# richardbaihe/a3t

Measured on AMD Instinct MI355X. Metric: mel-frames/sec (train), higher is better.
Workload: dtype bf16; 1 GPU; VCTK A3T masked-mel train step: 6+6 Conformer blocks d=384 H=2 ff=1536(k3), B=32/GPU, T_mel=1000, T_phn=120, postnet 5x256x5, fwd+bwd+clip+Adam, dropout 0.2/0.2/0.2 + postnet 0.5 (recipe); global_batch=32, parallelism=dp1, params=100799808

## Files before the change

a3t_amd/_lib.py:

```python
import ctypes
import os
from ctypes import POINTER, c_char_p, c_float, c_int, c_int32, c_int64, c_void_p

import torch

HERE = os.path.dirname(os.path.abspath(__file__))
LIB_PATH = os.environ.get("A3T_LIB_PATH") or os.path.join(HERE, "lib", "liba3t_hip.so")

F32, BF16 = 0, 1
ACT_NONE, ACT_RELU, ACT_TANH, ACT_SWISH = 0, 1, 2, 3
ACC_STORE, ACC_ADD, ACC_ATOMIC, ACC_SOLE = 0, 1, 2, 3


class GemmDesc(ctypes.Structure):
    _fields_ = [
        ("A", c_void_p), ("B", c_void_p), ("C", c_void_p), ("bias", c_void_p), ("R", c_void_p), ("S", c_void_p),
        ("M", c_int32), ("N", c_int32), ("K", c_int32),
        ("a_rs", c_int64), ("a_cs", c_int64),
        ("b_rs", c_int64), ("b_cs", c_int64), ("b_ts", c_int64),
        ("c_rs", c_int64),
        ("batch", c_int32), ("batch_inner", c_int32),
        ("a_bs0", c_int64), ("a_bs1", c_int64), ("b_bs0", c_int64), ("b_bs1", c_int64),
        ("c_bs0", c_int64), ("c_bs1", c_int64),
        ("taps", c_int32), ("pad", c_int32), ("dil", c_int32), ("Tseq", c_int32), ("kshift", c_int32),
# ... 35 lines not shown
    "a3t_attn_scale_rows": [_P, _P, _P, c_int, c_int, c_int, c_int, _P],
    "a3t_attn_bwd_ds": [_P, _P, _P, _P, _P, _P, _P, c_int, c_int, c_int, c_int, c_int64, c_int64, c_int64, c_int64, c_float,
                        c_float, ctypes.c_uint32, c_int, c_int64, _P],
    "a3t_attn_fwd": [_P, _P, _P, _P, _P, _P, _P, _P, c_int, c_int, c_int, c_int, c_int64, c_int64, c_int64, c_int64,
                     c_float, c_float, ctypes.c_uint32, _P, _P, _P],
    "a3t_pwg_block": [_P, _P, _P, _P, _P, _P, _P, _P, c_int, c_int, c_int, _P],
    "a3t_mask_fill": [_P, _P, _P, _P, c_int, c_int, c_int, _P],
    "a3t_embed_finish_fwd": [_P, _P, _P, _P, _P, _P, _P, c_int, c_int, c_int, c_int, c_float, c_float, ctypes.c_uint32,
                             _P, _P],
    "a3t_embed_finish_bwd": [_P, _P, _P, _P, _P, _P, _P, _P, c_int, c_int, c_int, c_int, c_int, c_int, c_float, c_float,
                             ctypes.c_uint32, _P],
    "a3t_scale": [_P, _P, c_int64, c_float, _P],
    "a3t_axpy": [_P, _P, c_int64, c_float, _P],
    "a3t_attn_bias_fold": [_P, c_int32, c_int32, _P, _P, _P, _P],
    "a3t_scale_dev": [_P, _P, c_int64, _P, _P],
    "a3t_slice_rows": [_P, _P, c_int, c_int, c_int, c_int, c_int, c_int, _P],
    "a3t_concat_rows": [_P, _P, _P, c_int, c_int, c_int, c_int, _P],
    "a3t_concat_rows_ragged": [_P, _P, _P, _P, _P, c_int, c_int, c_int, c_int, c_int64, c_int64, _P],
    "a3t_split_rows": [_P, _P, _P, c_int, c_int, c_int, c_int, _P],
    "a3t_cast_bf16": [_P, _P, c_int64, _P],
    "a3t_cast_bf16_conv_t": [_P, _P, _P, _P, c_int, c_int, c_int, c_int, _P],
    "a3t_split_bf16": [_P, _P, _P, c_int64, _P],
    "a3t_reflect_pad": [_P, _P, c_int, c_int, c_int, c_int, _P],
    "a3t_reflect_pad_ragged": [_P, _P, _P, c_int, c_int, c_int, c_int, _P],
    "a3t_stft_amp": [_P, _P, c_int64, c_int, c_int, _P],
    "a3t_logmel_finish": [_P, _P, c_int, c_int, c_int, _P],
    "a3t_mlm_loss": [_P, _P, _P, _P, _P, _P, _P, _P, c_int, c_int, c_int, c_float, _P],
    "a3t_mlm_loss_scratch_floats": [c_int],
    "a3t_sumsq": [_P, c_int64, _P, _P],
    "a3t_clip_adam": [_P, _P, _P, _P, _P, _P, c_int64, c_float, c_float, c_float, c_float, c_int, c_float, c_float,
                      _P],
    "a3t_clip_adam_noam": [_P, _P, _P, _P, _P, _P, c_int64, _P, c_float, c_float, c_float, c_float, c_float, c_float,
                           c_float, c_float, _P],
    "a3t_sgd_step": [_P, _P, c_int64, c_float, c_float, _P],
    "a3t_pwg_gate": [_P, _P, _P, c_int64, c_int, _P],
    "a3t_pwg_res_skip": [_P, _P, _P, c_int64, c_int, c_int, _P],
    "a3t_pwg_upsample": [_P, _P, _P, c_int64, c_int64, c_int, c_int, _P],
    "a3t_replicate_pad": [_P, _P, c_int64, c_int64, c_int, c_int, _P],
    "a3t_bias_act": [_P, _P, c_int64, c_int, c_int, c_float, _P],
    "a3t_replicate_pad_ragged": [_P, _P, _P, c_int64, c_int64, c_int, c_int, _P],
    "a3t_pwg_upsample_ragged": [_P, _P, _P, _P, c_int, c_int64, c_int64, c_int, c_int, _P],
    "a3t_zero_tail": [_P, _P, c_int, c_int64, c_int64, c_int, _P],
    "a3t_layernorm_fwd_ragged": [_P, _P, _P, _P, _P, _P, _P, c_int, c_int, c_int, c_float, _P],
    "a3t_glu_dwconv_fwd_ragged": [_P, _P, _P, _P, _P, _P, c_int, c_int, c_int, c_int, _P],
    "a3t_relpos_softmax_fwd_ragged": [_P, _P, c_int, _P, _P, c_int, c_int, c_int, c_int, c_int64, c_int64, c_int64, c_float,
                                      _P],
    "a3t_splice_spans": [_P, _P, _P, _P, _P, _P, c_int, c_int, c_int, c_int, _P],
    "a3t_pwg_block_ragged": [_P, _P, _P, _P, _P, _P, _P, _P, _P, c_int, c_int, c_int, c_int, _P],
    "a3t_pwg_block_f16": [_P, _P, _P, _P, _P, _P, _P, _P, _P, c_int, c_int, c_int, c_int, _P],
    "a3t_cast_f16_sat": [_P, _P, c_int64, _P],
    "a3t_hfg_conv": [_P, _P, _P, _P, _P, _P, c_float, c_int, c_float, _P, c_int, c_int, c_int, c_int, c_int, c_int, _P],
    "a3t_hfg_conv_f16": [_P, _P, _P, _P, _P, _P, c_float, c_int, c_float, _P, c_int, c_int, c_int, c_int, c_int, c_int, _P],
    "a3t_hfg_out": [_P, _P, _P, _P, c_float, _P, c_int, c_int, c_int, c_int, c_int, _P],
    "a3t_leaky_relu": [_P, _P, c_int64, c_float, _P],
    "a3t_mgan_stack": [_P, _P, _P, _P, c_float, _P, c_int, c_int, c_int, c_int, c_int, c_int, _P],
    "a3t_mgan_out": [_P, _P, _P, _P, c_float, c_int, _P, c_int, c_int, c_int, c_int, c_int, c_int, c_int, _P],
    "a3t_pqmf_synthesis": [_P, _P, _P, _P, c_int, c_int, c_int, c_int, c_int, _P],
    "a3t_reflect_pad_rows": [_P, _P, c_int64, c_int64, c_int, c_int, _P],
    "a3t_reflect_pad_rows_ragged": [_P, _P, _P, c_int, c_int64, c_int64, c_int, c_int, _P],
    "a3t_smg_conv": [_P, _P, _P, _P, _P, _P, _P, c_int, c_int, _P, c_int, c_int, c_int, c_int, c_int, c_int, c_int, c_int, c_int,
                     c_int, _P],
    "a3t_smg_stats": [_P, _P, _P, c_float, _P, c_int, c_int, c_int, c_int, _P],
    "a3t_duration_head": [_P, _P, _P, _P, _P, _P, _P, c_int, c_int, c_float, c_float, _P],
    "a3t_l2_normalize": [_P, _P, c_int, c_int, c_float, _P],
    "a3t_gst_conv_bn_relu": [_P, _P, _P, _P, _P, _P, c_int, c_int, c_int, c_int, c_int, c_int, c_int, _P],
    "a3t_gst_gru_stl": [_P, _P, _P, _P, _P, _P, _P, _P, _P, _P, _P, _P, c_int, c_int, c_int, c_int, c_int, c_int, _P],
# ... 57 lines not shown
```

a3t_amd/conformer.py:

```python
import math
import os
import zlib
from dataclasses import dataclass

import torch

from . import ops
from ._lib import ACC_ADD, ACC_ATOMIC, ACC_STORE, ACT_RELU, ACT_SWISH, BF16, F32
from .config import A3TConfig
from .params import ParamStore
from .schedule import StepSchedule


def legacy_pe_table(c: A3TConfig) -> torch.Tensor:
    d = c.adim
    position = torch.arange(c.max_len - 1, -1, -1.0, dtype=torch.float32).unsqueeze(1)
    div = torch.exp(torch.arange(0, d, 2, dtype=torch.float32) * -(math.log(10000.0) / d))
    pe = torch.zeros(c.max_len, d)
    pe[:, 0::2] = torch.sin(position * div)
    pe[:, 1::2] = torch.cos(position * div)
    return pe


def score_chunks(lengths, heads, max_score_elems):
    order = sorted(range(len(lengths)), key=lambda i: (lengths[i], i))
    out, cur = [], []
    for i in order:
        if cur and (len(cur) + 1) * heads * lengths[i] ** 2 > max_score_elems:
            out.append(cur)
            cur = []
        cur.append(i)
    if cur:
        out.append(cur)
    return out


@dataclass
class EngineOptions:
    side_stream: bool = True
    side2: bool = True
    side_depth: int = 48
    wgrad_group: bool = True
    post_f32_first: bool = True
    attn_bwd_ds: bool = True
    attn_signed: bool = True
    attn_dq_dual: bool = True
    attn_dbd_view: bool = True
    attn_dk_main: bool = True
    fused_attn: str = "auto"
    fused_attn_train: int = 1
    ffn_8p: bool = True
    ffn_keep4: bool = True
    lin_dgrad_t: bool = True
    fuse_ln_dropout: bool = True

    @classmethod
    def from_env(cls, environ=os.environ):
        fa, ft = environ.get("A3T_FUSED_ATTN", "auto"), environ.get("A3T_FUSED_ATTN_TRAIN", "1")
        if fa not in ("auto", "fwd", "0"):
            raise ValueError(f"A3T_FUSED_ATTN={fa!r}: expected auto, fwd or 0 (the flash backward behind '1' left the library in "
                             "round 5, tools/experiments/attn_flash_backward.patch)")
        on = {f: environ.get("A3T_" + f.upper(), "1") != "0" for f in
              ("side_stream", "side2", "wgrad_group", "post_f32_first", "attn_bwd_ds", "attn_signed", "attn_dq_dual",
               "attn_dbd_view", "attn_dk_main", "ffn_8p", "ffn_keep4", "lin_dgrad_t")}
        return cls(side_depth=max(2, int(environ.get("A3T_SIDE_DEPTH", "48"))), fused_attn=fa,
                   fused_attn_train=0 if ft == "0" else 2 if ft == "2" else 1, **on)


class ConformerStack(StepSchedule):
    def __init__(self, cfg: A3TConfig, store: ParamStore, compute: str = "f32", training: bool = True,
                 dropout: bool = False, options: EngineOptions = None):
        self.opt = opt = options if options is not None else EngineOptions.from_env()
        super().__init__(store.device, opt.side_stream, opt.side2, opt.side_depth)
        self.c = cfg
        self.dropping = bool(dropout and training)
        self.step_seed = 0
        self.store = store
        self.bf16 = (compute == "bf16")
        self.adt = torch.bfloat16 if self.bf16 else torch.float32
        self.cmp = BF16 if self.bf16 else F32
        self.training = training
        self.pe = legacy_pe_table(cfg).to(self.dev)
        self.sv = {}
        self.scratch64 = torch.zeros(4 * max(cfg.ff, 3 * cfg.adim, cfg.postnet_chans, 64), dtype=torch.float64,
                                     device=self.dev)
        self.bn_momentum = 0.1
        self._wg_group = 4 if (self.bf16 and self.side is not None and self._depth >= 8 and opt.wgrad_group) else 1
        self._wg_pending, self._wg_slots = [], set()
        self._gm_ready = None
        self.colsum_slots = 16
        self.fused_attn_fwd_only = self.bf16 and opt.fused_attn == "fwd"
        self.fused_attn_auto = self.bf16 and opt.fused_attn == "auto"
        self.fused_attn_train = self.bf16 and opt.fused_attn == "auto" and opt.fused_attn_train != 0
        self.fused_attn_train_min = 1 if opt.fused_attn_train == 2 else 64
        self._fused_now = self._fused_train_now = False
        self.attn_path, self.block_dims = {}, {}
        self._need_grad = training
        self._mode_tag = None
        if self.bf16:
            for n, v in (("adim", cfg.adim), ("ff", cfg.ff), ("idim", cfg.idim), ("odim", cfg.odim),
                         ("dk", cfg.dk), ("postnet_chans", cfg.postnet_chans or 8)):
                if v % 8:
                    raise ValueError(f"compute='bf16' needs {n} % 8 == 0 (16-byte DMA granules), got {v}")
            self.flat16 = torch.zeros(store.total, dtype=torch.bfloat16, device=self.dev)
            self.p16 = {k: self.flat16[o:o + math.prod(s)].view(s) for k, (o, s) in store.offsets.items()}
        self._ffn_plans = {}
        self._lin_plans = {}
        self._wt = {}
        self._P_ahead, self._pos_ev = {}, None
        self._cast_ev = self._wt_ev = None
        dec = [o for k, (o, _) in store.offsets.items() if k.startswith("dec.")]
        self._cast_split = min(dec) if dec else 0

    def _drop(self, p, tag):
        if not self.dropping or p <= 0.0:
            return None
        h = (zlib.crc32(tag.encode()) ^ ((self.step_seed * 0x9E3779B1) & 0xFFFFFFFF)) & 0xFFFFFFFF
        h = ((h ^ (h >> 16)) * 0x85EBCA6B) & 0xFFFFFFFF
        h = ((h ^ (h >> 13)) * 0xC2B2AE35) & 0xFFFFFFFF
        return (float(p), (h ^ (h >> 16)) & 0xFFFFFFFF)

    def _gm(self, g, tag, p, bias_grad, bias_scale):
        dr = self._drop(p, tag)
        if dr is None:
            return (self._g16(g) if self.bf16 else g)
        gm = self.ws.get(self._t("tmp.gm"), tuple(g.shape), self.adt)
        if self._gm_ready == tag:
            self._gm_ready = None
            return gm
        ops.dropout_bwd_cast(g, gm, dr[0], dr[1], colsum=bias_grad, colsum_scale=bias_scale)
        return gm

    def W(self, name):
        return self.p16[name] if self.bf16 else self.store.p[name]

    def refresh_weights(self):
        self._cast_ev = self._wt_ev = None
        if not self.bf16:
            return
        split = self._cast_split if self.side is not None else 0
        flat, flat16 = self.store.flat, self.flat16
        wt = list(self._wt.values()) if self._need_grad else []

        def transposed():
            for src_off, dst_off, _, tflat, shp in wt:
                ops.cast_bf16_conv_t(flat, tflat, src_off, dst_off, *shp)
        if split <= 0:
            ops.cast_bf16(flat, flat16)
            transposed()
            return
        ops.cast_bf16(flat[:split], flat16[:split])
        self._cast_ev = self._side(lambda: ops.cast_bf16(flat[split:], flat16[split:]), want_event="cast")
        if wt:
            self._wt_ev = self._side(transposed, want_event="wt")

    def _wait_cast(self, which):
        ev = getattr(self, which, None)
        if ev is not None:
            ev.wait_on(torch.cuda.current_stream())
            setattr(self, which, None)

    def _setup_wt(self, suf, shape):
        stored = (tuple(shape), (shape[0], shape[2])) if shape[1] == 1 else (tuple(shape),)
        names = [k for k in self.store.offsets if k.endswith("." + suf) and tuple(self.store.offsets[k][1]) in stored]
        if not names:
            return
        n = math.prod(shape)
        flat = torch.zeros(n * len(names), dtype=torch.bfloat16, device=self.dev)
        src = torch.tensor([self.store.offsets[k][0] for k in names], dtype=torch.int64, device=self.dev)
        dst = torch.arange(len(names), dtype=torch.int64, device=self.dev) * n
        views = {k: flat[i * n:(i + 1) * n].view(shape[2], shape[1], shape[0]) for i, k in enumerate(names)}
        self._wt[suf] = (src, dst, views, flat, tuple(shape))
        ops.cast_bf16_conv_t(self.store.flat, flat, src, dst, *shape)

    def _ffn_plan(self, M):
        key = (M, self._need_grad, self._mode_tag, self.opt.ffn_8p, self.opt.ffn_keep4)
        if key not in self._ffn_plans:
            c = self.c
            keep = d1 = d2 = keep4 = False
            if self._need_grad and self.bf16 and self.dev.type == "cuda" and self.opt.ffn_8p:
                k = c.ff_kernel
                drop = ops.G8_DROP if (self.dropping and c.dropout_rate > 0) else 0
                keep = ops.gemm_8p_supported(M, c.ff, k * c.adim, k, ops.G8_BIAS_ACT | drop | ops.G8_KEEP_OUT) and \
                    ops.gemm_8p_supported(M, c.ff, k * c.adim, k, ops.G8_KEEP_IN | ops.G8_COLSUM)
                d1 = ops.gemm_8p_supported(M, c.adim, k * c.ff, k, 0) or ops.gemm_pn_supported(M, c.adim, k * c.ff, k, 0)
                d2 = (not keep) and \
                    ops.gemm_pn_supported(M, c.ff, k * c.adim, k, ops.G8_SMASK | ops.G8_COLSUM)
                keep4 = (not keep) and self.opt.ffn_keep4 and c.ff % 8 == 0 and \
                    ops.gemm_pn_supported(M, c.ff, k * c.adim, k, ops.G8_KEEP_IN | ops.G8_COLSUM)
                d2 = d2 or keep4
                if (keep or d2) and "w2" not in self._wt:
                    self._setup_wt("w2", (c.adim, k, c.ff))
                if d1 and "w1" not in self._wt:
                    self._setup_wt("w1", (c.ff, k, c.adim))
                keep, d1, d2 = keep and "w2" in self._wt, d1 and "w1" in self._wt, d2 and "w2" in self._wt
                keep4 = keep4 and d2
            self._ffn_plans[key] = (keep, d1, d2, keep4)
# ... 472 lines not shown
```

a3t_amd/csrc/misc.hip:

```cpp
#include <hip/hip_runtime.h>
#include <math.h>
#include <stdint.h>
#include "../../include/a3t_hip.h"
#include "dtype_io.h"

static inline int nblocks(int64_t n, int cap = 4096) {
    int64_t b = (n + 255) / 256;
    return (int)(b > cap ? cap : (b < 1 ? 1 : b));
}
#define GRID_STRIDE(i, n) \
    for (int64_t i = (int64_t)blockIdx.x * blockDim.x + threadIdx.x; i < (n); i += (int64_t)gridDim.x * blockDim.x)

__global__ void mask_fill_kernel(const float* __restrict__ x, const uint8_t* __restrict__ m,
                                 const float* __restrict__ mf, void* __restrict__ y, int y_dt, int64_t n, int C) {
    GRID_STRIDE(i, n) {
        int64_t r = i / C;
        int c = (int)(i - r * C);
        stx(y, y_dt, i, m[r] ? mf[c] : x[i]);
    }
}
extern "C" int a3t_mask_fill(const float* speech, const uint8_t* masked, const float* mask_feature, void* out,
                             int out_dtype, int M, int C, void* stream) {
    int64_t n = (int64_t)M * C;
    hipLaunchKernelGGL(mask_fill_kernel, dim3(nblocks(n)), dim3(256), 0, (hipStream_t)stream, speech, masked,
// ... 480 lines not shown
    __shared__ double red[256];
    double s = 0.0;
    for (int i = threadIdx.x; i < SUMSQ_BLOCKS; i += 256) s += partial[i];
    red[threadIdx.x] = s;
    __syncthreads();
    for (int o = 128; o > 0; o >>= 1) {
        if (threadIdx.x < o) red[threadIdx.x] += red[threadIdx.x + o];
        __syncthreads();
    }
    const float norm = (float)sqrt(red[0]) * fabsf(gscale);
    if (blockIdx.x == 0 && threadIdx.x == 0) norm_out[0] = norm;
    if (!isfinite(norm)) return;
    const double t = (double)(state[0] + 1);
    const float lr = (float)((double)base_lr * pow((double)model_size, -0.5) * fmin(pow(t, -0.5), t * pow((double)warmup, -1.5)));
    const float bc1 = (float)(1.0 - pow((double)b1, t));
    const float bc2s = (float)sqrt(1.0 - pow((double)b2, t));
    float coef = clip > 0.f ? clip / (norm + 1e-6f) : 1.f;
    coef = (coef > 1.f ? 1.f : coef) * gscale;
    const float step_size = lr / bc1;
    adam_sweep(p, g, m, v, n, coef, b1, b2, step_size, bc2s, eps);
}
__global__ void adam_state_advance_kernel(const float* norm, int* state) {
    if (isfinite(norm[0])) state[0] += 1; else state[1] += 1;
}
extern "C" int a3t_clip_adam_noam(float* p, const float* g, float* m, float* v, const double* partial, float* norm_out,
                                  int64_t n, int* state, float base_lr, float model_size, float warmup, float beta1,
                                  float beta2, float eps, float clip, float gscale, void* stream) {
    hipLaunchKernelGGL(clip_adam_noam_kernel, dim3(nblocks(n / 4, 2048)), dim3(256), 0, (hipStream_t)stream, p, g, m, v,
                       partial, norm_out, n, state, base_lr, model_size, warmup, beta1, beta2, eps, clip, gscale);
    hipLaunchKernelGGL(adam_state_advance_kernel, dim3(1), dim3(1), 0, (hipStream_t)stream, norm_out, state);
    return (int)hipGetLastError();
}

__global__ __launch_bounds__(256) void sgd_step_kernel(float* __restrict__ p, const float* __restrict__ g, const int64_t n,
                                                       const float step) {
    const int64_t tid = (int64_t)blockIdx.x * blockDim.x + threadIdx.x, nthr = (int64_t)gridDim.x * blockDim.x;
    const bool vec = ((((uintptr_t)p) | ((uintptr_t)g)) & 15) == 0;
    const int64_t n4 = vec ? n / 4 : 0;
    for (int64_t i = tid; i < n4; i += nthr) {
        float4 pi = ((float4*)p)[i];
        const float4 gi = ((const float4*)g)[i];
        pi.x -= step * gi.x, pi.y -= step * gi.y, pi.z -= step * gi.z, pi.w -= step * gi.w;
        ((float4*)p)[i] = pi;
    }
    for (int64_t i = n4 * 4 + tid; i < n; i += nthr) p[i] -= step * g[i];
}
extern "C" int a3t_sgd_step(float* p, const float* g, int64_t n, float lr, float gscale, void* stream) {
    if (n <= 0) return 0;
    hipLaunchKernelGGL(sgd_step_kernel, dim3(nblocks((n + 3) / 4, 2048)), dim3(256), 0, (hipStream_t)stream, p, g, n,
                       lr * gscale);
    return (int)hipGetLastError();
}

__global__ void pwg_gate_kernel(const float* __restrict__ y, const float* __restrict__ c, float* __restrict__ out,
                                int64_t n, int H) {
    GRID_STRIDE(i, n) {
        int64_t t = i / H;
        int h = (int)(i - t * H);
        int64_t j = t * 2 * H + h;
        float a = y[j] + c[j], b = y[j + H] + c[j + H];
        out[i] = tanhf(a) * (1.f / (1.f + __expf(-b)));
    }
}
extern "C" int a3t_pwg_gate(const float* y, const float* c, float* out, int64_t T, int H, void* stream) {
    int64_t n = T * H;
    hipLaunchKernelGGL(pwg_gate_kernel, dim3(nblocks(n)), dim3(256), 0, (hipStream_t)stream, y, c, out, n, H);
// ... 259 lines not shown
```

a3t_amd/ops.py:

```python
import ctypes
import os

import torch

from . import _lib as L
from ._lib import ACC_ADD, ACC_ATOMIC, ACC_SOLE, ACC_STORE, ACT_NONE, ACT_RELU, ACT_SWISH, ACT_TANH, BF16, F32

__all__ = ["gemm", "gemm_plan", "linear_fwd", "linear_bwd_data", "linear_bwd_weight", "conv_fwd", "conv_bwd_data",
           "conv_bwd_weight"]


PROFILE = None


def _stream():
    return ctypes.c_void_p(torch.cuda.current_stream().cuda_stream)


def _ptr(t):
    if t is None:
        return None
    return ctypes.c_void_p(t.data_ptr())


# ... 423 lines not shown
    host_lens = [int(n) for n in host_lens]
    if len(host_lens) != B or lens.numel() != B:
        raise ValueError(f"reflect_pad_ragged: {B} rows, {len(host_lens)} host lengths, {lens.numel()} device lengths")
    for b, n in enumerate(host_lens):
        if n <= pad or n > N:
            raise ValueError(f"reflect_pad_ragged: row {b} has {n} samples; reflection by {pad} needs {pad} < n <= {N}")
    L.check(L.load().a3t_reflect_pad_ragged(_ptr(x), _ptr(out), _ptr(_i32(lens, "lens")), B, N, pad, out.shape[1], _stream()),
            "reflect_pad_ragged")


def stft_amp(S, amp, nbins):
    L.check(L.load().a3t_stft_amp(_ptr(S), _ptr(amp), amp.shape[0], nbins, amp.shape[1], _stream()), "stft_amp")


def logmel_finish(mel, olens, B, F, C):
    L.check(L.load().a3t_logmel_finish(_ptr(mel), _ptr(olens), B, F, C, _stream()), "logmel_finish")


def mlm_loss(before, after, target, masked, loss_out, d_before, d_after, scratch, l2=False, gscale=1.0):
    M, C = before.shape
    L.check(L.load().a3t_mlm_loss(_ptr(before), _ptr(after), _ptr(target), _ptr(masked), _ptr(loss_out),
                                  _ptr(d_before), _ptr(d_after), _ptr(scratch), M, C, int(l2), gscale, _stream()),
            "mlm_loss")


def loss_scratch_floats(M):
    return L.load().a3t_mlm_loss_scratch_floats(M)


def sumsq(g, partial):
    L.check(L.load().a3t_sumsq(_ptr(g), g.numel(), _ptr(partial), _stream()), "sumsq")


def clip_adam(p, g, m, v, partial, norm_out, lr, step, clip=1.0, gscale=1.0, betas=(0.9, 0.999), eps=1e-8):
    L.check(L.load().a3t_clip_adam(_ptr(p), _ptr(g), _ptr(m), _ptr(v), _ptr(partial), _ptr(norm_out), p.numel(), lr,
                                   betas[0], betas[1], eps, step, clip, gscale, _stream()), "clip_adam")


def clip_adam_noam(p, g, m, v, partial, norm_out, state, base_lr, model_size, warmup, clip=1.0, gscale=1.0,
                   betas=(0.9, 0.999), eps=1e-8):
    L.check(L.load().a3t_clip_adam_noam(_ptr(p), _ptr(g), _ptr(m), _ptr(v), _ptr(partial), _ptr(norm_out), p.numel(),
                                        _ptr(state), base_lr, float(model_size), float(warmup), betas[0], betas[1], eps,
                                        clip, gscale, _stream()), "clip_adam_noam")


def sgd_step(p, g, lr, gscale=1.0):
    if p.dtype != torch.float32 or g.dtype != torch.float32 or p.numel() != g.numel() or not (p.is_contiguous() and g.is_contiguous()):
        raise ValueError("sgd_step: p and g must be contiguous fp32 buffers of one size")
    L.check(L.load().a3t_sgd_step(_ptr(p), _ptr(g), p.numel(), float(lr), float(gscale), _stream()), "sgd_step")


def pwg_gate(y, c, out):
    T, H = out.shape
    L.check(L.load().a3t_pwg_gate(_ptr(y), _ptr(c), _ptr(out), T, H, _stream()), "pwg_gate")


def pwg_res_skip(o, x, skips):
    T, R = x.shape
    L.check(L.load().a3t_pwg_res_skip(_ptr(o), _ptr(x), _ptr(skips), T, R, skips.shape[1], _stream()), "pwg_res_skip")


def _i32(t, what):
    if t.dtype != torch.int32 or not t.is_contiguous():
        raise ValueError(f"{what} must be a contiguous int32 tensor")
    return t


def _rows_lens(what, x, lens):
    B = x.shape[0] if x.dim() == 3 else 1
    if lens is not None and _i32(lens, "lens").numel() != B:
        raise ValueError(f"{what}: {lens.numel()} lengths for {B} rows")
    return (B, *x.shape[-2:])


def pwg_upsample(c, w, out, scale_, lens=None, mul=1):
    B, Tin, C = _rows_lens("pwg_upsample", c, lens)
    if lens is None:
        rc = L.load().a3t_pwg_upsample(_ptr(c), _ptr(w), _ptr(out), B, Tin, C, scale_, _stream())
    else:
        rc = L.load().a3t_pwg_upsample_ragged(_ptr(c), _ptr(w), _ptr(out), _ptr(lens), mul, B, Tin, C, scale_, _stream())
    L.check(rc, "pwg_upsample")

# ... 393 lines not shown
```

a3t_amd/trainer.py:

```python
import os
from typing import Dict, List, Sequence

import torch
import torch.distributed as dist

from .config import A3TConfig


def shard_batches(batches: Sequence[Sequence[str]], rank: int, world: int) -> List[List[str]]:
    for b in batches:
        if len(b) < world:
            raise RuntimeError(f"The batch-size must be equal or more than world_size: {len(b)} < {world}")
    return [list(b[rank::world]) for b in batches]


def noam_lr(step: int, base_lr: float, model_size: int, warmup: int) -> float:
    return base_lr * model_size ** -0.5 * min(step ** -0.5, step * warmup ** -1.5)


def iterator_stop(local_done: bool, device="cpu") -> bool:
    if not (dist.is_available() and dist.is_initialized()):
        return local_done
    t = torch.tensor([1 if local_done else 0], dtype=torch.int64, device=device)
    dist.all_reduce(t, op=dist.ReduceOp.SUM)
# ... 64 lines not shown
    def wait(self):
        for w, rng in self.works:
            if rng is None:
                w.wait()
                continue
            if self.cuda:
                with torch.cuda.stream(self.stream):
                    w.wait()
                    self.g[rng[0]:rng[1]].copy_(self.stage[rng[0]:rng[1]])
            else:
                w.wait()
                self.g[rng[0]:rng[1]].copy_(self.stage[rng[0]:rng[1]])
        self.works = []
        if self.cuda:
            torch.cuda.current_stream().wait_stream(self.stream)


class A3TTrainer:

    def __init__(self, cfg: A3TConfig, store, compute="bf16", lr=1.0, warmup_steps=4000, grad_clip=1.0,
                 betas=(0.9, 0.999), eps=1e-8, overlap=True, dropout=True, force_reducer=False,
                 bucket_min_elems=16 * 1024 * 1024, comm_dtype=torch.float32):
        from .engine import MLMEngine
        self.cfg, self.store = cfg, store
        self.engine = MLMEngine(cfg, store, compute=compute, training=True, dropout=dropout)
        dev = store.device
        self.m = torch.zeros_like(store.flat)
        self.v = torch.zeros_like(store.flat)
        self.partial = torch.zeros(1024, dtype=torch.float64, device=dev)
        self.norm = torch.zeros(1, device=dev)
        self.step_no = 0
        self.opt_state = torch.zeros(2, dtype=torch.int32, device=dev)
        self.comm_dtype = comm_dtype
        self.lr, self.warmup, self.clip, self.betas, self.eps = lr, warmup_steps, grad_clip, betas, eps
        self.world = dist.get_world_size() if (dist.is_available() and dist.is_initialized()) else 1
        self._main = None
        if dev.type == "cuda":
            from .schedule import shared_stream
            self._main = shared_stream(dev, "main", high=True)
        self.reducer = None
        if self.world > 1 or (force_reducer and dist.is_available() and dist.is_initialized()):
            dist.broadcast(store.flat, 0)
            for b in store.buf.values():
                dist.broadcast(b, 0)
            bounds = [store.offsets[f"pre.{i}.ffm.ln.g"][0] for i in range(cfg.pre_blocks)]
            bounds += [store.offsets[f"enc.{i}.ffm.ln.g"][0] for i in range(cfg.enc_blocks)]
            bounds += [store.offsets[f"dec.{i}.ffm.ln.g"][0] for i in range(cfg.dec_blocks if cfg.has_decoder else 0)]
            bounds += [store.offsets["sfc.w"][0]]
            self.ranges = bucket_ranges(store.total, bounds, bucket_min_elems)
            if overlap:
                self.reducer = FlatAllReduce(store.grad, self.ranges, comm_dtype)

    def step(self, batch: Dict[str, torch.Tensor], total_weight: float = None, accum_grad: int = 1,
             accum_index: int = 0) -> torch.Tensor:
        if self._main is None:
            return self._step(batch, total_weight, accum_grad, accum_index)
        cur = torch.cuda.current_stream(self.store.device)
        self._main.wait_stream(cur)
        with torch.cuda.stream(self._main):
            loss = self._step(batch, total_weight, accum_grad, accum_index)
        cur.wait_stream(self._main)
        loss.record_stream(cur)
        return loss

    def _step(self, batch: Dict[str, torch.Tensor], total_weight: float = None, accum_grad: int = 1,
              accum_index: int = 0) -> torch.Tensor:
        from . import ops
        st = self.store
        if accum_index == 0:
            st.zero_grad()
        if self.engine.bf16:
            from .espnet_model import ESPnetMLMEncAsDecoderModel
            batch = ESPnetMLMEncAsDecoderModel._pad_to_dma_granule(batch)
        w = 1.0
        if total_weight is not None:
            w = grad_scale(float(batch["speech"].shape[0]), float(total_weight), self.world)
        out = self.engine.forward(batch, gscale=w / accum_grad)
        last = (accum_index == accum_grad - 1)
        if self.reducer is not None and last:
            self._backward_overlapped()
        else:
            self.engine.backward()
            if self.world > 1 and last:
                dist.all_reduce(st.grad)
        if not last:
            return out["loss"]
        self.step_no += 1
        ops.sumsq(st.grad, self.partial)
        ops.clip_adam_noam(st.flat, st.grad, self.m, self.v, self.partial, self.norm, self.opt_state, self.lr,
                           self.cfg.adim, self.warmup, clip=self.clip, gscale=1.0 / self.world, betas=self.betas,
                           eps=self.eps)
        return out["loss"]

    def optimizer_steps(self):
        a, sk = self.opt_state.tolist()
        if sk:
            import logging
            logging.warning(f"{sk} step(s) had a non-finite gradient norm and were skipped (trainer.py:640-645)")
        return a, sk

    def _backward_overlapped(self):
        eng, red = self.engine, self.reducer
        state = {"next": 0}
        lows = [lo for lo, _ in red.ranges]
        offs = self.store.offsets

        def after(name):
            lo = offs[name][0]
            if state["next"] < len(lows) and lows[state["next"]] >= lo and hasattr(eng, "join_side"):
                eng.join_side()
            while state["next"] < len(lows) and lows[state["next"]] >= lo:
                red.reduce_range(state["next"])
                state["next"] += 1

        eng.backward(on_group_done=after)
        while state["next"] < len(lows):
            red.reduce_range(state["next"])
            state["next"] += 1
        red.wait()

    def state(self):
        applied = int(self.opt_state[0])
        return dict(model=self.store.state_dict(), optimizers=[dict(m=self.m.cpu(), v=self.v.cpu(), step=applied)],
                    schedulers=[dict(step=applied, warmup_steps=self.warmup)], reporter=None, scaler=None)
# ... 10 lines not shown
```

include/a3t_hip.h:

```cpp
#ifndef A3T_HIP_H
#define A3T_HIP_H
#include <stdint.h>

#ifdef __cplusplus
extern "C" {
#endif

#define A3T_F32 0
#define A3T_BF16 1

#define A3T_EINVAL (-22)

#define A3T_ACT_NONE 0
#define A3T_ACT_RELU 1
#define A3T_ACT_TANH 2
#define A3T_ACT_SWISH 3

#define A3T_ACC_STORE 0
#define A3T_ACC_ADD 1
#define A3T_ACC_ATOMIC 2
#define A3T_ACC_SOLE 3

typedef struct a3t_gemm_desc {
    const void* A;
// ... 104 lines not shown
int a3t_axpy(const float* x, float* y, int64_t n, float a, void* stream);
int a3t_attn_bias_fold(const float* slots, int S, int d, float* gu, float* gv, float* gbqkv, void* stream);
int a3t_scale_dev(const float* x, float* y, int64_t n, const float* s, void* stream);
int a3t_slice_rows(const float* x, void* y, int y_dtype, int B, int T, int Tm, int D, int reverse_add,
                   void* stream);
int a3t_concat_rows(const float* speech, const float* text, float* xs, int B, int Tm, int Tp, int D, void* stream);
int a3t_split_rows(const float* dxs, float* dspeech, float* dtext, int B, int Tm, int Tp, int D, void* stream);
int a3t_concat_rows_ragged(const float* speech, const float* text, float* xs, const int32_t* slens, const int32_t* tlens, int B,
                           int Tm, int Tp, int D, int64_t speech_bs, int64_t text_bs, void* stream);
int a3t_cast_bf16(const float* x, void* y, int64_t n, void* stream);
int a3t_cast_bf16_conv_t(const float* src, void* dst, const int64_t* src_off, const int64_t* dst_off, int count, int N,
                         int taps, int C, void* stream);
int a3t_split_bf16(const float* x, void* hi, void* lo, int64_t n, void* stream);

int a3t_reflect_pad(const float* x, float* out, int B, int N, int pad, int ld, void* stream);
int a3t_reflect_pad_ragged(const float* x, float* out, const int32_t* lens, int B, int N, int pad, int ld, void* stream);
int a3t_stft_amp(const float* S, float* amp, int64_t rows, int nbins, int ld, void* stream);
int a3t_logmel_finish(float* mel, const int64_t* olens, int B, int F, int C, void* stream);

int a3t_mlm_loss(const float* before, const float* after, const float* target, const uint8_t* masked,
                 float* loss_out, float* d_before, float* d_after, float* scratch, int M, int C, int l2,
                 float gscale, void* stream);
int a3t_mlm_loss_scratch_floats(int M);

int a3t_sumsq(const float* g, int64_t n, double* partial , void* stream);
int a3t_clip_adam(float* p, const float* g, float* m, float* v, const double* partial, float* norm_out,
                  int64_t n, float lr, float beta1, float beta2, float eps, int step, float clip,
                  float gscale, void* stream);

int a3t_clip_adam_noam(float* p, const float* g, float* m, float* v, const double* partial, float* norm_out, int64_t n,
                       int32_t* state, float base_lr, float model_size, float warmup, float beta1, float beta2,
                       float eps, float clip, float gscale, void* stream);

int a3t_sgd_step(float* p, const float* g, int64_t n, float lr, float gscale, void* stream);

int a3t_pwg_gate(const float* y, const float* c, float* out, int64_t T, int H, void* stream);
int a3t_pwg_res_skip(const float* o, float* x, float* skips, int64_t T, int R, int S, void* stream);
int a3t_pwg_upsample(const float* c, const float* w, float* out, int64_t B, int64_t Tin, int C, int scale,
                     void* stream);
int a3t_replicate_pad(const float* x, float* y, int64_t B, int64_t T, int C, int pad, void* stream);
int a3t_bias_act(float* x, const float* bias, int64_t M, int C, int act, float scale, void* stream);
int a3t_replicate_pad_ragged(const float* x, float* y, const int32_t* lens, int64_t B, int64_t T, int C, int pad,
                             void* stream);
int a3t_pwg_upsample_ragged(const float* c, const float* w, float* out, const int32_t* lens, int mul, int64_t B,
                            int64_t Tin, int C, int scale, void* stream);
int a3t_zero_tail(float* x, const int32_t* lens, int mul, int64_t B, int64_t T, int C, void* stream);
int a3t_layernorm_fwd_ragged(const float* x, const float* gamma, const float* beta, float* y, float* mean, float* rstd,
                             const int32_t* lens, int B, int T, int D, float eps, void* stream);
int a3t_glu_dwconv_fwd_ragged(const float* g, const float* wdw, const float* bdw, float* glu, float* z, const int32_t* lens,
                              int B, int Tseq, int C, int K, void* stream);
int a3t_relpos_softmax_fwd_ragged(const void* ac, const void* bd, int scores_dtype, const int32_t* lens, void* probs,
                                  int probs_dtype, int B, int H, int T, int64_t ac_bs, int64_t bd_bs, int64_t p_bs,
                                  float scale, void* stream);
int a3t_splice_spans(const float* after, const float* speech, const uint8_t* speech_mask, const int32_t* spans, float* out,
                     int32_t* lens, int B, int Tin, int Tout, int C, void* stream);

int a3t_duration_head(const float* z, const float* gamma, const float* beta, const float* w, const float* bias,
                      float* logd, int64_t* frames, int M, int C, float eps, float offset, void* stream);
int a3t_l2_normalize(const float* x, float* y, int B, int n, float eps, void* stream);

int a3t_gst_conv_bn_relu(const float* x, const float* w, const float* scale, const float* shift, float* y,
                         const int32_t* lens, int B, int Tin, int Fin, int Cin, int Cout, int k, int s, void* stream);
int a3t_gst_gru_stl(const float* gi, const float* w_hh, const float* b_hh, const int32_t* lens, const float* w_q,
                    const float* b_q, const float* k_tok, const float* v_tok, const float* w_out, const float* b_out,
                    float* ref_embs, float* style, int B, int T, int H, int d, int heads, int tokens, void* stream);
int a3t_gst_add_style(float* hs, const float* style, const int32_t* rows, int B, int T, int d, int S, void* stream);
// ... 71 lines not shown
```

Measured before the change: 780,200 mel-frames/s.

## Fuse bf16 weight shadow and transposed-weight casts into the Adam update kernel

The Adam step now writes the bf16 copy of each parameter and the transposed/tap-reversed bf16 weight shadows straight from registers, using a tile table that maps flat regions to transposed destinations. The next step's separate cast and transpose pass is skipped when a version token shows the fp32 buffer is unchanged since the optimizer wrote it. This removes one full read of the fp32 parameter buffer and extra kernel launches each step. In exchange it adds an LDS-tiled transpose inside the optimizer kernel, host-side table validation, and staleness tracking through tensor version counters.

```diff
diff --git a/a3t_amd/_lib.py b/a3t_amd/_lib.py
--- a/a3t_amd/_lib.py
+++ b/a3t_amd/_lib.py
@@ -91,6 +91,9 @@
                       _P],
     "a3t_clip_adam_noam": [_P, _P, _P, _P, _P, _P, c_int64, _P, c_float, c_float, c_float, c_float, c_float, c_float,
                            c_float, c_float, _P],
+    "a3t_adam_shadow_table": [_P, c_int, c_int64, _P],
+    "a3t_clip_adam_noam_shadow": [_P, _P, _P, _P, _P, _P, c_int64, _P, c_float, c_float, c_float, c_float, c_float, c_float,
+                                  c_float, c_float, _P, _P, _P, c_int, _P],
     "a3t_sgd_step": [_P, _P, c_int64, c_float, c_float, _P],
     "a3t_pwg_gate": [_P, _P, _P, c_int64, c_int, _P],
     "a3t_pwg_res_skip": [_P, _P, _P, c_int64, c_int, c_int, _P],
diff --git a/a3t_amd/conformer.py b/a3t_amd/conformer.py
--- a/a3t_amd/conformer.py
+++ b/a3t_amd/conformer.py
@@ -53,6 +53,7 @@
     ffn_keep4: bool = True
     lin_dgrad_t: bool = True
     fuse_ln_dropout: bool = True
+    adam_shadows = True
 
     @classmethod
     def from_env(cls, environ=os.environ):
@@ -63,8 +64,47 @@
         on = {f: environ.get("A3T_" + f.upper(), "1") != "0" for f in
               ("side_stream", "side2", "wgrad_group", "post_f32_first", "attn_bwd_ds", "attn_signed", "attn_dq_dual",
                "attn_dbd_view", "attn_dk_main", "ffn_8p", "ffn_keep4", "lin_dgrad_t")}
-        return cls(side_depth=max(2, int(environ.get("A3T_SIDE_DEPTH", "48"))), fused_attn=fa,
-                   fused_attn_train=0 if ft == "0" else 2 if ft == "2" else 1, **on)
+        opt = cls(side_depth=max(2, int(environ.get("A3T_SIDE_DEPTH", "48"))), fused_attn=fa,
+                  fused_attn_train=0 if ft == "0" else 2 if ft == "2" else 1, **on)
+        opt.adam_shadows = environ.get("A3T_ADAM_SHADOWS", "1") != "0"
+        return opt
+
+
+def shadow_group_names(offsets, suf, shape):
+    stored = (tuple(shape), (shape[0], shape[2])) if shape[1] == 1 else (tuple(shape),)
+    return [k for k in offsets if k.endswith("." + suf) and tuple(offsets[k][1]) in stored]
+
+
+def shadow_set_id(wt):
+    return tuple((suf, id(g[3])) for suf, g in wt.items())
+
+
+def shadow_regions(offsets, wt):
+    out = []
+    for _, _, views, tflat, (N, taps, C) in wt.values():
+        for i, name in enumerate(views):
+            out.append((offsets[name][0], tflat, i * N * taps * C, N, taps, C))
+    return sorted(out, key=lambda r: r[0])
+
+
+def shadow_remainder(regions, total):
+    out, end = [], 0
+    for src, _, _, N, taps, C in regions:
+        if src > end:
+            out.append((end, src))
+        end = src + N * taps * C
+    if total > end:
+        out.append((end, total))
+    return out
+
+
+class ShadowToken:
+
+    def __init__(self, flat, set_id):
+        self.ptr, self.version, self.set_id = flat.data_ptr(), flat._version, set_id
+
+    def valid(self, flat, set_id):
+        return self.ptr == flat.data_ptr() and self.version == flat._version and self.set_id == set_id
 
 
 class ConformerStack(StepSchedule):
@@ -109,6 +149,7 @@
         self._wt = {}
         self._P_ahead, self._pos_ev = {}, None
         self._cast_ev = self._wt_ev = None
+        self._fresh = None
         dec = [o for k, (o, _) in store.offsets.items() if k.startswith("dec.")]
         self._cast_split = min(dec) if dec else 0
 
@@ -138,6 +179,9 @@
         self._cast_ev = self._wt_ev = None
         if not self.bf16:
             return
+        if self.shadows_fresh():
+            return
+        self._fresh = None
         split = self._cast_split if self.side is not None else 0
         flat, flat16 = self.store.flat, self.flat16
         wt = list(self._wt.values()) if self._need_grad else []
@@ -154,6 +198,13 @@
         if wt:
             self._wt_ev = self._side(transposed, want_event="wt")
 
+    def shadows_written(self):
+        self._fresh = ShadowToken(self.store.flat, shadow_set_id(self._wt))
+
+    def shadows_fresh(self):
+        return bool(self.bf16 and self.opt.adam_shadows and self._fresh is not None and
+                    self._fresh.valid(self.store.flat, shadow_set_id(self._wt)))
+
     def _wait_cast(self, which):
         ev = getattr(self, which, None)
         if ev is not None:
@@ -161,8 +212,7 @@
             setattr(self, which, None)
 
     def _setup_wt(self, suf, shape):
-        stored = (tuple(shape), (shape[0], shape[2])) if shape[1] == 1 else (tuple(shape),)
-        names = [k for k in self.store.offsets if k.endswith("." + suf) and tuple(self.store.offsets[k][1]) in stored]
+        names = shadow_group_names(self.store.offsets, suf, shape)
         if not names:
             return
         n = math.prod(shape)
diff --git a/a3t_amd/csrc/misc.hip b/a3t_amd/csrc/misc.hip
--- a/a3t_amd/csrc/misc.hip
+++ b/a3t_amd/csrc/misc.hip
@@ -536,6 +536,187 @@
     return (int)hipGetLastError();
 }
 
+#define SHT 64
+enum { SH_SRC = 0, SH_DST, SH_DOFF, SH_N, SH_TAPS, SH_C, SH_FLAT0, SH_TILE0 };
+static_assert(A3T_SHADOW_COLS == 8 && A3T_SHADOW_FLAT == 4096, "table row, flat tile = 256 lanes x 4 float4");
+static inline int64_t sh_cdiv(int64_t a, int64_t b) { return (a + b - 1) / b; }
+static bool shadow_row(const int64_t* e, bool closing, int64_t n, int64_t& end, int64_t& tile) {
+    const int64_t src = e[SH_SRC], N = e[SH_N], taps = e[SH_TAPS], C = e[SH_C];
+    if (src < end || src % 4 || src > n) return false;
+    if (e[SH_FLAT0] != end || e[SH_TILE0] != tile) return false;
+    tile += sh_cdiv(src - end, A3T_SHADOW_FLAT);
+    if (closing) return src == n && !N && !taps && !C;
+    if (N <= 0 || taps <= 0 || C <= 0 || C % 4 || N > INT32_MAX || taps > INT32_MAX || C > INT32_MAX) return false;
+    if (N * taps > (n - src) / C) return false;
+    if (!e[SH_DST] || (e[SH_DST] & 1) || e[SH_DOFF] < 0) return false;
+    tile += sh_cdiv(N, SHT) * taps * sh_cdiv(C, SHT);
+    end = src + N * taps * C;
+    return true;
+}
+static int64_t shadow_table_tiles(const int64_t* tb, int count, int64_t n) {
+    if (!tb || count < 0 || n <= 0 || n % 4) return -1;
+    int64_t end = 0, tile = 0;
+    for (int r = 0; r <= count; ++r)
+        if (!shadow_row(tb + (int64_t)r * A3T_SHADOW_COLS, r == count, n, end, tile)) return -1;
+    return tile;
+}
+extern "C" int a3t_adam_shadow_table(const int64_t* regions, int count, int64_t n, int64_t* table) {
+    if ((!regions && count) || !table || count < 0 || n <= 0 || n % 4) return A3T_EINVAL;
+    int64_t end = 0, tile = 0;
+    for (int r = 0; r <= count; ++r) {
+        int64_t* e = table + (int64_t)r * A3T_SHADOW_COLS;
+        for (int j = 0; j < 6; ++j) e[j] = r < count ? regions[(int64_t)r * 6 + j] : 0;
+        if (r == count) e[SH_SRC] = n;
+        e[SH_FLAT0] = end, e[SH_TILE0] = tile;
+        if (!shadow_row(e, r == count, n, end, tile)) return A3T_EINVAL;
+    }
+    return 0;
+}
+__device__ __forceinline__ void adam_elem4(float4& p, const float4 g, float4& m, float4& v, const float coef, const float b1,
+                                           const float b2, const float step_size, const float bc2s, const float eps) {
+    adam_elem(p.x, g.x, m.x, v.x, coef, b1, b2, step_size, bc2s, eps);
+    adam_elem(p.y, g.y, m.y, v.y, coef, b1, b2, step_size, bc2s, eps);
+    adam_elem(p.z, g.z, m.z, v.z, coef, b1, b2, step_size, bc2s, eps);
+    adam_elem(p.w, g.w, m.w, v.w, coef, b1, b2, step_size, bc2s, eps);
+}
+__device__ __forceinline__ uint2 pack4(const float4 v) {
+    uint2 o;
+    o.x = io_pack2(v.x, v.y);
+    o.y = io_pack2(v.z, v.w);
+    return o;
+}
+__global__ __launch_bounds__(256) void clip_adam_noam_shadow_kernel(float* __restrict__ p, const float* __restrict__ g,
+                                                                    float* __restrict__ m, float* __restrict__ v,
+                                                                    const double* partial, float* norm_out,
+                                                                    unsigned short* __restrict__ flat16,
+                                                                    const int64_t* __restrict__ tb, int count, int64_t ntiles,
+                                                                    const int* state, float base_lr, float model_size,
+                                                                    float warmup, float b1, float b2, float eps, float clip,
+                                                                    float gscale) {
+    __shared__ double red[256];
+    __shared__ float tile[SHT][SHT + 1];
+    double s = 0.0;
+    for (int i = threadIdx.x; i < SUMSQ_BLOCKS; i += 256) s += partial[i];
+    red[threadIdx.x] = s;
+    __syncthreads();
+    for (int o = 128; o > 0; o >>= 1) {
+        if (threadIdx.x < o) red[threadIdx.x] += red[threadIdx.x + o];
+        __syncthreads();
+    }
+    const float norm = (float)sqrt(red[0]) * fabsf(gscale);
+    if (blockIdx.x == 0 && threadIdx.x == 0) norm_out[0] = norm;
+    if (!isfinite(norm)) return;
+    const double t = (double)(state[0] + 1);
+    const float lr = (float)((double)base_lr * pow((double)model_size, -0.5) * fmin(pow(t, -0.5), t * pow((double)warmup, -1.5)));
+    const float bc1 = (float)(1.0 - pow((double)b1, t));
+    const float bc2s = (float)sqrt(1.0 - pow((double)b2, t));
+    float coef = clip > 0.f ? clip / (norm + 1e-6f) : 1.f;
+    coef = (coef > 1.f ? 1.f : coef) * gscale;
+    const float step_size = lr / bc1;
+
+    const int64_t t0 = ntiles * blockIdx.x / gridDim.x, t1 = ntiles * (blockIdx.x + 1) / gridDim.x;
+    if (t0 >= t1) return;
+    int r = 0;
+    for (int lo = 0, hi = count; lo <= hi;) {
+        const int mid = (lo + hi) >> 1;
+        if (tb[(int64_t)mid * A3T_SHADOW_COLS + SH_TILE0] <= t0) r = mid, lo = mid + 1; else hi = mid - 1;
+    }
+    const int tid = threadIdx.x;
+    for (int64_t tl = t0; tl < t1; ++tl) {
+        while (r < count && tb[(int64_t)(r + 1) * A3T_SHADOW_COLS + SH_TILE0] <= tl) ++r;
+        const int64_t* e = tb + (int64_t)r * A3T_SHADOW_COLS;
+        const int64_t src = e[SH_SRC], flat0 = e[SH_FLAT0];
+        const int64_t treg = e[SH_TILE0] + (src - flat0 + A3T_SHADOW_FLAT - 1) / A3T_SHADOW_FLAT;
+        if (tl < treg) {
+            const int64_t i0 = (flat0 >> 2) + (tl - e[SH_TILE0]) * (A3T_SHADOW_FLAT / 4), iend = src >> 2;
+            float4 pi[4], gi[4], mi[4], vi[4];
+#pragma unroll
+            for (int k = 0; k < 4; ++k) {
+                const int64_t i = i0 + tid + 256 * k;
+                if (i < iend) pi[k] = ((float4*)p)[i], gi[k] = ((const float4*)g)[i], mi[k] = ((float4*)m)[i], vi[k] = ((float4*)v)[i];
+            }
+#pragma unroll
+            for (int k = 0; k < 4; ++k) {
+                const int64_t i = i0 + tid + 256 * k;
+                if (i < iend) {
+                    adam_elem4(pi[k], gi[k], mi[k], vi[k], coef, b1, b2, step_size, bc2s, eps);
+                    ((float4*)m)[i] = mi[k], ((float4*)v)[i] = vi[k], ((float4*)p)[i] = pi[k];
+                    ((uint2*)flat16)[i] = pack4(pi[k]);
+                }
+            }
+            continue;
+        }
+        const int N = (int)e[SH_N], taps = (int)e[SH_TAPS], C = (int)e[SH_C];
+        unsigned short* Wt = (unsigned short*)e[SH_DST] + e[SH_DOFF];
+        const int tc = (C + SHT - 1) / SHT;
+        int64_t q = tl - treg;
+        const int c0 = (int)(q % tc) * SHT;
+        q /= tc;
+        const int tap = (int)(q % taps), n0 = (int)(q / taps) * SHT;
+        {
+            const int c = c0 + 4 * (tid & 15), ry = tid >> 4;
+            float4 pi[4], gi[4], mi[4], vi[4];
+#pragma unroll
+            for (int k = 0; k < 4; ++k) {
+                const int nn = n0 + ry + 16 * k;
+                if (nn < N && c < C) {
+                    const int64_t i = (src + ((int64_t)nn * taps + tap) * C + c) >> 2;
+                    pi[k] = ((float4*)p)[i], gi[k] = ((const float4*)g)[i], mi[k] = ((float4*)m)[i], vi[k] = ((float4*)v)[i];
+                }
+            }
+#pragma unroll
+            for (int k = 0; k < 4; ++k) {
+                const int nn = n0 + ry + 16 * k;
+                if (nn < N && c < C) {
+                    const int64_t i = (src + ((int64_t)nn * taps + tap) * C + c) >> 2;
+                    adam_elem4(pi[k], gi[k], mi[k], vi[k], coef, b1, b2, step_size, bc2s, eps);
+                    ((float4*)m)[i] = mi[k], ((float4*)v)[i] = vi[k], ((float4*)p)[i] = pi[k];
+                    ((uint2*)flat16)[i] = pack4(pi[k]);
+                    float* row = &tile[ry + 16 * k][4 * (tid & 15)];
+                    row[0] = pi[k].x, row[1] = pi[k].y, row[2] = pi[k].z, row[3] = pi[k].w;
+                }
+            }
+        }
+        __syncthreads();
+        {
+            const bool vec8 = (N % 8 == 0) && (((uintptr_t)Wt & 15) == 0);
+            const int j0 = 8 * (tid & 7), nn = n0 + j0;
+#pragma unroll
+            for (int k = 0; k < 2; ++k) {
+                const int cl = (tid >> 3) + 32 * k, c = c0 + cl;
+                if (c >= C || nn >= N) continue;
+                unsigned short* o = Wt + ((int64_t)c * taps + (taps - 1 - tap)) * N + nn;
+                if (vec8) {
+                    uint4 w;
+                    w.x = io_pack2(tile[j0 + 0][cl], tile[j0 + 1][cl]);
+                    w.y = io_pack2(tile[j0 + 2][cl], tile[j0 + 3][cl]);
+                    w.z = io_pack2(tile[j0 + 4][cl], tile[j0 + 5][cl]);
+                    w.w = io_pack2(tile[j0 + 6][cl], tile[j0 + 7][cl]);
+                    *(uint4*)o = w;
+                } else {
+                    for (int j = 0; j < 8 && nn + j < N; ++j) o[j] = io_f2bf(tile[j0 + j][cl]);
+                }
+            }
+        }
+        __syncthreads();
+    }
+}
+extern "C" int a3t_clip_adam_noam_shadow(float* p, const float* g, float* m, float* v, const double* partial, float* norm_out,
+                                         int64_t n, int32_t* state, float base_lr, float model_size, float warmup, float beta1,
+                                         float beta2, float eps, float clip, float gscale, void* flat16,
+                                         const int64_t* table_host, const int64_t* table_dev, int count, void* stream) {
+    if (!p || !g || !m || !v || !flat16 || !table_dev) return A3T_EINVAL;
+    if (((((uintptr_t)p) | ((uintptr_t)g) | ((uintptr_t)m) | ((uintptr_t)v)) & 15) || ((uintptr_t)flat16 & 7)) return A3T_EINVAL;
+    const int64_t ntiles = shadow_table_tiles(table_host, count, n);
+    if (ntiles <= 0) return A3T_EINVAL;
+    const int grid = (int)(ntiles < 2048 ? ntiles : 2048);
+    hipLaunchKernelGGL(clip_adam_noam_shadow_kernel, dim3(grid), dim3(256), 0, (hipStream_t)stream, p, g, m, v, partial,
+                       norm_out, (unsigned short*)flat16, table_dev, count, ntiles, state, base_lr, model_size, warmup, beta1,
+                       beta2, eps, clip, gscale);
+    hipLaunchKernelGGL(adam_state_advance_kernel, dim3(1), dim3(1), 0, (hipStream_t)stream, norm_out, state);
+    return (int)hipGetLastError();
+}
+
 __global__ __launch_bounds__(256) void sgd_step_kernel(float* __restrict__ p, const float* __restrict__ g, const int64_t n,
                                                        const float step) {
     const int64_t tid = (int64_t)blockIdx.x * blockDim.x + threadIdx.x, nthr = (int64_t)gridDim.x * blockDim.x;
diff --git a/a3t_amd/ops.py b/a3t_amd/ops.py
--- a/a3t_amd/ops.py
+++ b/a3t_amd/ops.py
@@ -479,9 +479,14 @@
     L.check(L.load().a3t_sumsq(_ptr(g), g.numel(), _ptr(partial), _stream()), "sumsq")
 
 
+def _wrote(t):
+    torch.autograd.graph.increment_version(t)
+
+
 def clip_adam(p, g, m, v, partial, norm_out, lr, step, clip=1.0, gscale=1.0, betas=(0.9, 0.999), eps=1e-8):
     L.check(L.load().a3t_clip_adam(_ptr(p), _ptr(g), _ptr(m), _ptr(v), _ptr(partial), _ptr(norm_out), p.numel(), lr,
                                    betas[0], betas[1], eps, step, clip, gscale, _stream()), "clip_adam")
+    _wrote(p)
 
 
 def clip_adam_noam(p, g, m, v, partial, norm_out, state, base_lr, model_size, warmup, clip=1.0, gscale=1.0,
@@ -489,12 +494,42 @@
     L.check(L.load().a3t_clip_adam_noam(_ptr(p), _ptr(g), _ptr(m), _ptr(v), _ptr(partial), _ptr(norm_out), p.numel(),
                                         _ptr(state), base_lr, float(model_size), float(warmup), betas[0], betas[1], eps,
                                         clip, gscale, _stream()), "clip_adam_noam")
+    _wrote(p)
+
+
+class AdamShadowTable:
+    COLS = 8
+
+    def __init__(self, regions, n, device):
+        self.regions = [tuple(r) for r in regions]
+        self.n = int(n)
+        self.dsts = [r[1] for r in self.regions]
+        rows = [[int(r[0]), r[1].data_ptr(), int(r[2]), int(r[3]), int(r[4]), int(r[5])] for r in self.regions]
+        reg = torch.tensor(rows, dtype=torch.int64).reshape(len(rows), 6).contiguous()
+        self.host = torch.zeros((len(rows) + 1) * self.COLS, dtype=torch.int64)
+        L.check(L.load().a3t_adam_shadow_table(_ptr(reg), len(rows), self.n, _ptr(self.host)), "adam_shadow_table")
+        self.dev = self.host.to(device)
+
+    def __len__(self):
+        return len(self.regions)
+
+
+def clip_adam_noam_shadow(p, g, m, v, partial, norm_out, state, base_lr, model_size, warmup, flat16, table, clip=1.0,
+                          gscale=1.0, betas=(0.9, 0.999), eps=1e-8):
+    if flat16.dtype != torch.bfloat16 or flat16.numel() != p.numel() or table.n != p.numel():
+        raise ValueError("clip_adam_noam_shadow: flat16 and the table must cover the parameter buffer")
+    L.check(L.load().a3t_clip_adam_noam_shadow(_ptr(p), _ptr(g), _ptr(m), _ptr(v), _ptr(partial), _ptr(norm_out), p.numel(),
+                                               _ptr(state), base_lr, float(model_size), float(warmup), betas[0], betas[1],
+                                               eps, clip, gscale, _ptr(flat16), _ptr(table.host), _ptr(table.dev),
+                                               len(table), _stream()), "clip_adam_noam_shadow")
+    _wrote(p)
 
 
 def sgd_step(p, g, lr, gscale=1.0):
     if p.dtype != torch.float32 or g.dtype != torch.float32 or p.numel() != g.numel() or not (p.is_contiguous() and g.is_contiguous()):
         raise ValueError("sgd_step: p and g must be contiguous fp32 buffers of one size")
     L.check(L.load().a3t_sgd_step(_ptr(p), _ptr(g), p.numel(), float(lr), float(gscale), _stream()), "sgd_step")
+    _wrote(p)
 
 
 def pwg_gate(y, c, out):
diff --git a/a3t_amd/trainer.py b/a3t_amd/trainer.py
--- a/a3t_amd/trainer.py
+++ b/a3t_amd/trainer.py
@@ -120,6 +120,7 @@
         self.step_no = 0
         self.opt_state = torch.zeros(2, dtype=torch.int32, device=dev)
         self.comm_dtype = comm_dtype
+        self._shadow_table = None
         self.lr, self.warmup, self.clip, self.betas, self.eps = lr, warmup_steps, grad_clip, betas, eps
         self.world = dist.get_world_size() if (dist.is_available() and dist.is_initialized()) else 1
         self._main = None
@@ -175,9 +176,20 @@
             return out["loss"]
         self.step_no += 1
         ops.sumsq(st.grad, self.partial)
-        ops.clip_adam_noam(st.flat, st.grad, self.m, self.v, self.partial, self.norm, self.opt_state, self.lr,
-                           self.cfg.adim, self.warmup, clip=self.clip, gscale=1.0 / self.world, betas=self.betas,
-                           eps=self.eps)
+        eng = self.engine
+        if eng.bf16 and eng.opt.adam_shadows and st.flat.is_cuda:
+            from .conformer import shadow_regions, shadow_set_id
+            sid = shadow_set_id(eng._wt)
+            if self._shadow_table is None or self._shadow_table[0] != sid:
+                self._shadow_table = (sid, ops.AdamShadowTable(shadow_regions(st.offsets, eng._wt), st.total, st.device))
+            ops.clip_adam_noam_shadow(st.flat, st.grad, self.m, self.v, self.partial, self.norm, self.opt_state, self.lr,
+                                      self.cfg.adim, self.warmup, eng.flat16, self._shadow_table[1], clip=self.clip,
+                                      gscale=1.0 / self.world, betas=self.betas, eps=self.eps)
+            eng.shadows_written()
+        else:
+            ops.clip_adam_noam(st.flat, st.grad, self.m, self.v, self.partial, self.norm, self.opt_state, self.lr,
+                               self.cfg.adim, self.warmup, clip=self.clip, gscale=1.0 / self.world, betas=self.betas,
+                               eps=self.eps)
         return out["loss"]
 
     def optimizer_steps(self):
diff --git a/include/a3t_hip.h b/include/a3t_hip.h
--- a/include/a3t_hip.h
+++ b/include/a3t_hip.h
@@ -160,6 +160,14 @@
                        int32_t* state, float base_lr, float model_size, float warmup, float beta1, float beta2,
                        float eps, float clip, float gscale, void* stream);
 
+#define A3T_SHADOW_COLS 8
+#define A3T_SHADOW_FLAT 4096
+int a3t_adam_shadow_table(const int64_t* regions, int count, int64_t n, int64_t* table);
+int a3t_clip_adam_noam_shadow(float* p, const float* g, float* m, float* v, const double* partial, float* norm_out, int64_t n,
+                              int32_t* state, float base_lr, float model_size, float warmup, float beta1, float beta2,
+                              float eps, float clip, float gscale, void* flat16, const int64_t* table_host,
+                              const int64_t* table_dev, int count, void* stream);
+
 int a3t_sgd_step(float* p, const float* g, int64_t n, float lr, float gscale, void* stream);
 
 int a3t_pwg_gate(const float* y, const float* c, float* out, int64_t T, int H, void* stream);
```

Measured after the change: 784,600 mel-frames/s (median of 6 runs). Within noise of the previous version (+0.6%).
